# MaxRamgraber/Triangular-Transport-Toolbox

Hardware: AMD Instinct MI355X
Metric: map-evals/sec (forward+inverse, N samples x D comps) (higher is better)
Workload: dtype f64; 1 GPU; C5: d=40 banded separable map, order 3, N=1e6 (Gaussian-mixture target); N_per_gpu=1000000, D=40, columns=40, inverse=table, layout=column-major resident in HBM, coefficients=reference-optimised (tests/golden), world_size=1

## Files before the change

### triangular_transport_toolbox_amd/build.py

```python
import hashlib
import os
import shlex
import shutil
import subprocess

PKG = os.path.dirname(os.path.abspath(__file__))
CSRC = os.path.join(PKG, 'csrc')
LIB = os.environ.get('TTM_BUILD_LIB') or os.path.join(PKG, 'libttm.so')
SOURCES = ['ttm_kernels.hip', 'ttm_band.hip', 'ttm_int.hip', 'ttm_optim.cpp', 'ttm_comm.cpp']
HEADERS = ['ttm_eval.h', 'ttm_math.h', 'ttm_vec.h', 'ttm_erf_table.h', 'ttm_uform.h', 'ttm_cheb_table.h', 'ttm_lbfgsb.h', 'ttm_bfgs.h', 'ttm_rng.h', 'ttm_band.h', 'ttm_band_etab.h', 'ttm_dev.h', 'ttm_dense.h', 'ttm_dense_table.h', 'ttm_int.h', 'ttm_xprog.h', 'ttm_handover.h', 'ttm_options.h',
           os.path.join('..', '..', 'include', 'ttm.h')]
FLAGS = ['-O3', '-std=c++17', '--offload-arch=gfx950', '-ffp-contract=off', '-fPIC', '-shared',
         '-DNDEBUG'] + shlex.split(os.environ.get('TTM_BUILD_FLAGS', ''))
LINK = ['-ldl', '-pthread']


def hipcc_path():
    for cand in (shutil.which('hipcc'), '/opt/rocm/bin/hipcc'):
        if cand and os.path.exists(cand):
            return cand
    raise RuntimeError('hipcc not found: the MI355X engine needs the ROCm toolchain to build libttm.so')


def _sources():
    return [os.path.join(CSRC, s) for s in SOURCES if os.path.exists(os.path.join(CSRC, s))]
# ... 96 lines not shown
```

### triangular_transport_toolbox_amd/csrc/ttm_band.h

```cpp
#pragma once

#include <stdint.h>

#include "../../include/ttm.h"

namespace ttm_band {

int build_records(const ttm_program* p, double* U, void* stream);

int record_stride(int cls, int lag);

bool usable(const ttm_program* p, int k0, int k1);

int forward(const ttm_program* p, const double* U, int k0, int k1, const double* Xsoa, int64_t ldx, int64_t N, double* Zsoa,
            int64_t ldz, double* logdet, const double* sigma, double* sumsq, int cus, size_t lds_per_cu, int block, void* stream, const char** kernel_name);

int inverse(const ttm_program* p, const double* U, int k0, int k1, const double* Zsoa, int64_t ldz, double* Xsoa, int64_t ldx,
            int64_t N, const double* tab_x, int T, const double* y_affine, const double* tmin, const double* tmax, const int32_t* bkt,
            int nb, const double* img, int img_doubles, int cus, size_t lds_per_cu, int window, int block, void* stream, const char** kernel_name);

int newton(const ttm_program* p, const double* U, int k0, int k1, const double* Zsoa, int64_t ldz, double* Xsoa, int64_t ldx, int64_t N,
           int32_t* iters, int cus, size_t lds_per_cu, int block, void* stream, const char** kernel_name);

int bisect(const ttm_program* p, const double* U, int k0, int k1, const double* Zsoa, int64_t ldz, double* Xsoa, int64_t ldx, int64_t N,
           int32_t* iters, int cus, size_t lds_per_cu, int block, void* stream, const char** kernel_name);

bool bisect_plans(const ttm_program* p, const double* U, int k0, int k1, const double* Zsoa, int64_t ldz, double* Xsoa, int64_t ldx, int64_t N,
                  int32_t* iters, int cus, size_t lds_per_cu, int block);

int roundtrip(const ttm_program* p, const double* U, int k0, int k1, const double* Xsoa, int64_t ldx, int64_t N, double* Zsoa, int64_t ldz,
              double* Xr, int64_t ldr, double* logdet, const double* sigma, double* sumsq, const double* tab_x, int T, const double* y_affine,
              const double* tmin, const double* tmax, const int32_t* bkt, int nb, int cus, size_t lds_per_cu, bool force, void* stream,
              const char** kernel_name);

// ... 6 lines not shown
```

### triangular_transport_toolbox_amd/csrc/ttm_band.hip

```cpp
#include <hip/hip_runtime.h>
#include <math.h>
#include <stdint.h>
#include <stdlib.h>
#include <type_traits>

#include "ttm_band.h"
#include "ttm_band_etab.h"
#include "ttm_band_image.h"

namespace ttm_band {

typedef const __attribute__((address_space(4))) double* cdbl_p;
typedef const __attribute__((address_space(4))) int* cint_p;
struct __attribute__((aligned(16))) D2 { double x, y; };

__device__ const double g_band_etab[2 * TTM_BAND_ET_N] = { TTM_BAND_ETAB_VALUES };
__device__ double g_band_taylor[6] = {1.0 / 5040.0, 1.0 / 720.0, 1.0 / 120.0, 1.0 / 24.0, 1.0 / 6.0, 0.5};

__host__ __device__ constexpr int cls_db(int cls) { return cls == 1 ? 3 : (cls == 2 ? 5 : (cls == 3 ? 7 : 10)); }
__host__ __device__ constexpr int cls_da(int cls) { return cls == 1 ? 1 : (cls == 2 ? 5 : (cls == 3 ? 7 : 10)); }
__host__ __device__ constexpr int cls_gs(int cls) { return cls == 1 ? 8 : (cls == 2 ? 16 : 24); }
__host__ __device__ constexpr int cls_gp(int cls) { return cls_db(cls) + 1 + cls_da(cls); }
__host__ __device__ constexpr int rec_stride(int cls, int lag) { return (TTM_P_HDR + lag * cls_gp(cls) + 7) / 8 * 8; }

#define BAND_ET_DOUBLES (2 * TTM_BAND_ET_N)
#define BAND_CT 1024
#define BAND_NS 4
#define BAND_PF 1

__device__ __forceinline__ void band_dma16(const void* g, unsigned int lds_wave_base) {
    asm volatile("s_mov_b32 m0, %1\n\ts_nop 0\n\tglobal_load_lds_dwordx4 %0, off" ::"v"(g), "s"(lds_wave_base) : "m0");
}
__device__ __forceinline__ unsigned int band_lds_addr(const void* p) {
    return (unsigned int)(uintptr_t)(const __attribute__((address_space(3))) void*)p;
}

template <bool WAIT = true>
__device__ __forceinline__ void band_stage(double* lds_dst, const double* src, int n) {
    const int units = n >> 1;
    const unsigned int base = band_lds_addr(lds_dst);
    for (int u0 = 0; u0 < units; u0 += BAND_CT) {
        const int u = u0 + (int)threadIdx.x;
        if (u < units) band_dma16(src + 2 * (size_t)u, __builtin_amdgcn_readfirstlane(base + (unsigned int)(u0 + ((int)threadIdx.x & ~63)) * 16u));
// ... 56 lines not shown
    if (k >= 0) {
        const double* h = hot(k);
        const int* uc = ucomp + k * TTM_UC_LEN;
        double* tab = U + uc[TTM_UC_TAB_OFF];
        for (int c = t; c < uc[TTM_UC_NI]; c += 64) tab[c * TTM_U_TSTRIDE + 12] = fma(2.0, h[3], -(double)(2 * c - 1));
    }
}

template <bool NT>
__device__ __forceinline__ void band_store2(char* p, double a, double b) {
    typedef double v2 __attribute__((ext_vector_type(2)));
    const v2 v = {a, b};
    if (NT) __builtin_nontemporal_store(v, (v2*)p);
    else *(v2*)p = v;
}
__device__ __forceinline__ D2 band_load2(const char* p) {
    typedef double v2 __attribute__((ext_vector_type(2)));
    const v2 v = *(const v2*)p;
    const D2 r = {v.x, v.y};
    return r;
}

__device__ __forceinline__ int band_med3(int v, int lo, int hi) {
    int r;
    asm("v_med3_i32 %0, %1, %2, %3" : "=v"(r) : "v"(v), "v"(lo), "s"(hi));
    return r;
}
__device__ __forceinline__ double band_absmin(double x, double hi) {
    double r;
    asm("v_min_f64 %0, |%1|, %2" : "=v"(r) : "v"(x), "s"(hi));
    return r;
}

__device__ __forceinline__ double band_expq(const double* etab, double x, cdbl_p kt) {
    const double xe = band_absmin(x, TTM_BAND_ET_XMAX);
    const unsigned int i = (unsigned int)(int)fma(xe, TTM_BAND_ET_INV_STEP, 0.5);
// ... 48 lines not shown
}

__device__ __forceinline__ double band_spline(const double* tab, int nI, double sp_a, double sp_b, double sp_ds, double x) {
    const int col = band_med3((int)fma(x, sp_b, sp_a), 0, nI - 1);
    const double* cp = (const double*)((const char*)tab + __umul24((unsigned int)col, TTM_U_TSTRIDE * 8));
    double c[12];
#pragma unroll
    for (int i = 0; i < 12; i += 2) { const D2 v = *(const D2*)(cp + i); c[i] = v.x; c[i + 1] = v.y; }
    const double s = fma(x, sp_ds, cp[12]);
    double m = c[11];
#pragma unroll
    for (int i = 10; i >= 0; --i) m = fma(m, s, c[i]);
    return m;
}

template <int CLS, int LAG, bool FULL, bool OWN>
__device__ __forceinline__ void band_forward_tile(cdbl_p P, cdbl_p kt, const double* etab, const double* tabs, int tab0, int kb, int ke,
                                                  const char* xcol, int64_t ldxb, char* zcol, int64_t ldzb, unsigned int tbase,
                                                  const unsigned int (&roff)[BAND_NS / 2], unsigned int c1_32,
                                                  double (&pend)[BAND_NS][LAG]) {
    constexpr int DB = cls_db(CLS), DA = cls_da(CLS), PS = rec_stride(CLS, LAG);
    constexpr int NS = BAND_NS, NP = NS / 2, HALF = 2 * BAND_CT;
    constexpr int PF = BAND_PF, RING = PF + 1;
    D2 xr[RING][NP];
#pragma unroll
    for (int i = 0; i < PF; ++i) {
        const char* xc0 = xcol + (int64_t)(kb + i < ke ? i : 0) * ldxb;
#pragma unroll
        for (int q = 0; q < NP; ++q) xr[i][q] = band_load2(xc0 + roff[q]);
    }
    cdbl_p rec = P + (int64_t)(kb + LAG) * PS;
    auto step = [&](int j, const D2 (&xc)[NP], D2 (&xn)[NP]) {
        {
            const char* xnext = j + PF < ke ? xcol + PF * ldxb : xcol;
#pragma unroll
            for (int q = 0; q < NP; ++q) xn[q] = band_load2(xnext + roff[q]);
        }
        __builtin_amdgcn_sched_barrier(0);
        const double start = rec[0], sp_a = rec[2], sp_b = rec[3], sp_ds = rec[4];
        const double own1 = OWN ? rec[7] : 0.0;
        cint_p ri = (cint_p)rec;
        const int nI = ri[10];
        const double* tab = tabs + (ri[11] - tab0);
#pragma unroll
        for (int q = 0; q < NP; ++q) {
            double zv[2];
#pragma unroll
            for (int h = 0; h < 2; ++h) {
                const int e = 2 * q + h;
                const double x = h ? xc[q].y : xc[q].x;
                const double m = (!OWN || nI > 0) ? band_spline(tab, nI, sp_a, sp_b, sp_ds, x) : 0.0;
                const double E = band_expq(etab, x, kt);
                zv[h] = OWN ? fma(own1, x, pend[e][0] + m) : pend[e][0] + m;
                band_push<DB, DA, LAG>(rec + TTM_P_HDR, start, x, E, pend[e]);
            }
            const unsigned int n = tbase + (unsigned int)(q * HALF);
            const D2 o = {zv[0], zv[1]};
            char* zp = zcol + (size_t)(n * 8u);
            if (FULL || n + 1 < c1_32) band_store2<false>(zp, o.x, o.y);
            else if (n < c1_32) *(double*)zp = o.x;
            __builtin_amdgcn_sched_barrier(0);
        }
        rec += PS; xcol += ldxb; zcol += ldzb;
    };
    int j = kb;
    for (; j + RING <= ke; j += RING) {
#pragma unroll
        for (int i = 0; i < RING; ++i) step(j + i, xr[i], xr[(i + PF) % RING]);
    }
#pragma unroll
    for (int i = 0; i < RING - 1; ++i)
        if (j + i < ke) step(j + i, xr[i], xr[(i + PF) % RING]);
}

__device__ __forceinline__ double band_log(double x) {
    int e;
// ... 397 lines not shown
                    lv[h] = fma((double)pexp[e], 6.93147180559945286e-01, band_log(prod[e]));
                    lv[h] = dmin[e] < 0.0 ? NAN : lv[h];
                    if (last) lv[h] += luni;
                }
                if (!first) {
                    if (n + 1 < c1_32) { const D2 o = *(const D2*)(logdet + n); lv[0] += o.x; lv[1] += o.y; }
                    else if (n < c1_32) lv[0] += logdet[n];
                }
                if (n + 1 < c1_32) band_store2<false>((char*)(logdet + n), lv[0], lv[1]);
                else if (n < c1_32) logdet[n] = lv[0];
            }
        }
    }
}

template <int CLS, int LAG, bool OWN>
__global__ __launch_bounds__(BAND_CT) void k_band_forward(const double* __restrict__ U_, int64_t p_off, int k0, int k1, int kcol0,
                                                          const double* __restrict__ X, int64_t ldx, int64_t N,
                                                          double* __restrict__ Z, int64_t ldz, int64_t rows_per_wg, int Bc) {
    constexpr int DB = cls_db(CLS), DA = cls_da(CLS), PS = rec_stride(CLS, LAG);
    constexpr int NS = BAND_NS, NP = NS / 2, CT = BAND_CT, ROWS = NS * CT, HALF = 2 * CT;
    extern __shared__ __align__(16) double g_lds[];
    double* etab = g_lds;
    double* tabs = g_lds + BAND_ET_DOUBLES;
    const int tid = threadIdx.x;
    const int64_t c0 = (int64_t)blockIdx.x * rows_per_wg;
    if (c0 >= N) return;
    const int64_t c1 = c0 + rows_per_wg < N ? c0 + rows_per_wg : N;
    const int ntile = (int)((c1 - c0 + ROWS - 1) / ROWS);
    band_stage<false>(etab, g_band_etab, 2 * TTM_BAND_ET_N);
    cdbl_p P = (cdbl_p)(U_ + p_off);
// ... 35 lines not shown
                for (int i = 0; i < LAG; ++i) {
                    const int cc = colb - LAG + i;
                    cdbl_p rec = P + (int64_t)(kb + i) * PS;
                    const char* col = (const char*)X + (int64_t)(cc < 0 ? 0 : cc) * ldxb;
#pragma unroll
                    for (int q = 0; q < NP; ++q) {
                        D2 xv = *(const D2*)(col + roff[q]);
                        if (cc < 0) { xv.x = 0.0; xv.y = 0.0; }
                        band_push<DB, DA, LAG>(rec + TTM_P_HDR, rec[0], xv.x, band_expq(etab, xv.x, kt), pend[2 * q]);
                        band_push<DB, DA, LAG>(rec + TTM_P_HDR, rec[0], xv.y, band_expq(etab, xv.y, kt), pend[2 * q + 1]);
                    }
                }
            }
            const char* xcol = (const char*)X + (int64_t)colb * ldxb;
            char* zcol = (char*)Z + (int64_t)(kb - k0) * ldzb;
            if (full) band_forward_tile<CLS, LAG, true, OWN>(P, kt, etab, tabs, tab0, kb, ke, xcol, ldxb, zcol, ldzb, tbase, roff, c1_32, pend);
            else band_forward_tile<CLS, LAG, false, OWN>(P, kt, etab, tabs, tab0, kb, ke, xcol, ldxb, zcol, ldzb, tbase, roff, c1_32, pend);
        }
    }
}

#define BAND_FEW_NS 2
#define BAND_FEW_TAB (4 * BAND_CT)
template <int CLS, int LAG, int LAGE, bool PLAIN, bool DENS>
__global__ __launch_bounds__(BAND_CT) void k_band_few(const double* __restrict__ U_, int64_t p_off, int k0, int k1, int kcol0,
                                                      const double* __restrict__ X, int64_t ldx, int64_t N,
                                                      double* __restrict__ Z, int64_t ldz, double* __restrict__ logdet,
                                                      const double* __restrict__ sigma, double* __restrict__ sumsq, int ntiles,
                                                      int tab0, int ntab) {
    constexpr int DB = cls_db(CLS), DA = cls_da(CLS), GP = cls_gp(CLS), PS = rec_stride(CLS, LAG);
    constexpr int NS = BAND_FEW_NS, NP = NS / 2, CT = BAND_CT, ROWS = NS * CT, HALF = 2 * CT, FD = TTM_P_FEW_D;
    extern __shared__ __align__(16) double g_lds[];
// ... 218 lines not shown
};

__device__ __forceinline__ void band_ring_fill(const double* img, int ncomp, double* tabs, int tab_slot, int n) {
    const int U = tab_slot >> 1;
    const int total = n * U;
    for (int u0 = 0; u0 < total; u0 += BAND_CT) {
        const int u = u0 + (int)threadIdx.x;
        if (u < total) {
            const int t = u / U, o = u - t * U;
            band_dma16(img + (size_t)(t % ncomp) * tab_slot + 2 * o,
                       __builtin_amdgcn_readfirstlane(band_lds_addr(tabs) + (unsigned int)(u0 + ((int)threadIdx.x & ~63)) * 16u));
        }
    }
}

template <int CLS, int LAG, bool RING = false, int G = 0>
__device__ __forceinline__ void band_inverse_tile(const BandInvCtx& cx, bool full, int kb, int ke, const char* zcol, char* xcol, unsigned int tbase,
                                                  const unsigned int (&roff)[BAND_NS / 2], double (&pend)[BAND_NS][LAG],
                                                  const D2 (&zfirst)[BAND_NS / 2], bool have_first, BandRing* rg = nullptr) {
    constexpr int DB = cls_db(CLS), DA = cls_da(CLS), PS = rec_stride(CLS, LAG);
    constexpr int NS = BAND_NS, NP = NS / 2, HALF = 2 * BAND_CT;
    cdbl_p rec = cx.P + (int64_t)(kb + LAG) * PS;
    cdbl_p kt = cx.kt;
    const double* slot = RING ? cx.tabs + (size_t)rg->pos * cx.tab_slot : cx.tabs;
    const double ystep = cx.ystep;
    const int nb1 = cx.nb - 1;
    D2 za[NP], zb[NP];
    if (have_first) {
#pragma unroll
        for (int q = 0; q < NP; ++q) za[q] = zfirst[q];
    } else {
#pragma unroll
        for (int q = 0; q < NP; ++q) za[q] = band_load2(zcol + roff[q]);
    }
    auto interp = [&](double y_lo, double x_lo, double x_hi, double e_lo, double tgt, double& rr, double& ee) {
        const double dx = fmax(x_hi - x_lo, 1e-300);
        double rc = __builtin_amdgcn_rcp(dx);
        rc = fma(fma(-dx, rc, 1.0), rc, rc);
        const double delta = (ystep * rc) * (tgt - x_lo);
        rr = delta + y_lo;
        const double w = (delta * -0.25) * (y_lo + rr);
        double p = fma(kt[0], w, kt[1]);
        p = fma(p, w, kt[2]);
        p = fma(p, w, kt[3]);
        p = fma(p, w, kt[4]);
        p = fma(p, w, kt[5]);
        p = fma(p, w, 1.0);
        p = fma(p, w, 1.0);
        ee = e_lo * p;
    };
    auto step = [&](int j, const D2 (&zc)[NP], D2 (&zn)[NP]) {
        {
            const char* znext = j + 1 < ke ? zcol + cx.ldzb : zcol;
#pragma unroll
            for (int q = 0; q < NP; ++q) zn[q] = band_load2(znext + roff[q]);
        }
        double start = rec[1];
        double gc[LAG * (DB + 1 + DA)];
#pragma unroll
        for (int i = 0; i < LAG * (DB + 1 + DA); ++i) gc[i] = rec[TTM_P_HDR + i];
        asm volatile("" : "+s"(start));
#pragma unroll
        for (int i = 0; i < LAG * (DB + 1 + DA); ++i) asm volatile("" : "+s"(gc[i]));
        __builtin_amdgcn_sched_barrier(0);
        double wl, wh, scale, bias;
        { const D2 a = *(const D2*)slot; wl = a.x; wh = a.y; const D2 b = *(const D2*)(slot + 2); scale = b.x; bias = b.y; }
        const lds_p xsl = band_lds(slot + BAND_RT_HDR) - 8 * cx.w0;
        const lds_p bkl = band_lds(slot + BAND_RT_HDR + cx.Weven);
        const bool deg = __builtin_amdgcn_readfirstlane(((const int*)slot)[10]) != 0;
        const int per = __builtin_amdgcn_readfirstlane(((const int*)slot)[8]);
// ... 55 lines not shown
                    int a = 0, b = cx.T;
                    while (a < b) {
                        const int mid = (a + b) >> 1;
                        if (xg[mid] < t) a = mid + 1; else b = mid;
                    }
                    const int i = min(max(a, 1), cx.T - 1);
                    interp(fma((double)i, ystep, cx.y0m), xg[i - 1], xg[i], band_expq_series((double)(i - 1) * ystep + cx.y0), t, r[e], E[e]);
                }
            }
        }
#pragma unroll
        for (int e = 0; e < NS; ++e) band_push<DB, DA, LAG>(gc, start, r[e], E[e], pend[e]);
        if (full) {
#pragma unroll
            for (int q = 0; q < NP; ++q) {
                band_store2<false>(xcol + (size_t)((tbase + (unsigned int)(q * HALF)) * 8u), r[2 * q], r[2 * q + 1]);
            }
        } else {
#pragma unroll
            for (int q = 0; q < NP; ++q) {
                const unsigned int n = tbase + (unsigned int)(q * HALF);
                const D2 o = {r[2 * q], r[2 * q + 1]};
                char* xp = xcol + (size_t)(n * 8u);
                if (n + 1 < cx.c1_32) *(D2*)xp = o;
                else if (n < cx.c1_32) *(double*)xp = o.x;
            }
        }
        rec += PS; slot += cx.tab_slot; zcol += cx.ldzb; xcol += cx.ldxb;
        if (RING) {
            if (++rg->pos == rg->R) { rg->pos = 0; slot = cx.tabs; }
            if (G > 0 && ++rg->gcnt == G) {
                rg->gcnt = 0;
                static_assert(G == 0 || G == 4, "the counted wait below is 3 G - 2");
                asm volatile("s_waitcnt vmcnt(10)" ::: "memory");
                __syncthreads();
            }
        }
    };
    int j = kb;
// ... 150 lines not shown
                    for (int q = 0; q < NP; ++q) {
                        D2 xv = {0.0, 0.0};
                        if (cc >= 0) xv = *(const D2*)(col + roff[q]);
                        band_push<DB, DA, LAG>(rec + TTM_P_HDR, rec[1], xv.x, cc >= 0 ? band_expq_series(xv.x) : 1.0, pend[2 * q]);
                        band_push<DB, DA, LAG>(rec + TTM_P_HDR, rec[1], xv.y, cc >= 0 ? band_expq_series(xv.y) : 1.0, pend[2 * q + 1]);
                    }
                }
            }
            const char* zcol = (const char*)Z + (int64_t)(kb - k0) * ldzb;
            char* xcol = (char*)X + (int64_t)colb * ldxb;
            band_inverse_tile<CLS, LAG>(cx, full, kb, ke, zcol, xcol, tbase, roff, pend, zfirst, tile == 0);
        }
    }
}

template <int CLS, int LAG, int G>
__global__ __launch_bounds__(BAND_CT) void k_band_inverse_ring(const double* __restrict__ U_, int64_t p_off, int k0, int k1, int kcol0,
                                                               const double* __restrict__ Z, int64_t ldz, double* X, int64_t ldx, int64_t N,
                                                               const double* __restrict__ tab_x, int T, double y0, double ystep, double ylast,
                                                               const double* __restrict__ tmin, const double* __restrict__ tmax,
                                                               const double* __restrict__ img, int nb, int tab_slot, int R,
                                                               int64_t rows_per_wg, int w0, int W) {
    constexpr int DB = cls_db(CLS), DA = cls_da(CLS), PS = rec_stride(CLS, LAG);
    constexpr int NS = BAND_NS, NP = NS / 2, CT = BAND_CT, ROWS = NS * CT, HALF = 2 * CT;
    extern __shared__ __align__(16) double g_lds[];
    const int tid = threadIdx.x;
    const int64_t c0 = (int64_t)blockIdx.x * rows_per_wg;
    if (c0 >= N) return;
    const int64_t c1 = c0 + rows_per_wg < N ? c0 + rows_per_wg : N;
    const int ntile = (int)((c1 - c0 + ROWS - 1) / ROWS);
    const int ncomp = k1 - k0;
// ... 12 lines not shown
    cx.y0 = y0; cx.ystep = ystep; cx.y0m = y0m; cx.ldzb = ldzb; cx.ldxb = ldxb; cx.c1_32 = (unsigned int)c1;
    BandRing rg;
    {
        const int U = tab_slot >> 1, nw = (U + 63) >> 6;
        const int piece = (tid >> 6) % nw;
        const int start = 64 * piece < U - 64 ? 64 * piece : U - 64;
        rg.src = (const char*)img + (size_t)(start + (tid & 63)) * 16;
        rg.dst = __builtin_amdgcn_readfirstlane((unsigned int)start * 16u);
        rg.tabs_lds = band_lds_addr(tabs);
        rg.stride = (unsigned int)tab_slot * 8u;
        rg.R = R; rg.ncomp = ncomp; rg.pos = 0; rg.gcnt = 0;
        rg.tpos = G > 0 ? R - G : 0;
        rg.tcomp = G > 0 ? (R - G) % ncomp : 0;
    }
    D2 zfirst[NP];
#pragma unroll
    for (int q = 0; q < NP; ++q) {
        unsigned int n = (unsigned int)c0 + 2u * (unsigned int)tid + (unsigned int)(q * HALF);
        n = n < last_pair ? n : last_pair;
        zfirst[q] = band_load2((const char*)Z + (size_t)(n * 8u));
    }
    band_ring_fill(img, ncomp, tabs, tab_slot, R);
    for (int i = tid; i < W; i += CT) {
        etab[2 * i] = band_expq_series(w0 + i == T - 1 ? ylast : (double)(w0 + i) * ystep + y0);
        etab[2 * i + 1] = fma((double)(w0 + i + 1), ystep, y0m);
    }
    asm volatile("s_waitcnt vmcnt(0)" ::: "memory");
    __syncthreads();
    for (int tile = 0; tile < ntile; ++tile) {
        const unsigned int tbase = (unsigned int)c0 + (unsigned int)tile * (unsigned int)ROWS + 2u * (unsigned int)tid;
        const bool full = c0 + (int64_t)(tile + 1) * ROWS <= c1;
        unsigned int roff[NP];
#pragma unroll
        for (int q = 0; q < NP; ++q) {
            unsigned int n = tbase + (unsigned int)(q * HALF);
            n = n < last_pair ? n : last_pair;
// ... 4 lines not shown
        for (int e = 0; e < NS; ++e)
#pragma unroll
            for (int l = 0; l < LAG; ++l) pend[e][l] = 0.0;
        for (int i = 0; i < LAG; ++i) {
            const int cc = kcol0 - LAG + i;
            cdbl_p rec = P + (int64_t)(k0 + i) * PS;
            const char* col = (const char*)X + (int64_t)(cc < 0 ? 0 : cc) * ldxb;
#pragma unroll
            for (int q = 0; q < NP; ++q) {
                D2 xv = {0.0, 0.0};
                if (cc >= 0) xv = *(const D2*)(col + roff[q]);
                band_push<DB, DA, LAG>(rec + TTM_P_HDR, rec[1], xv.x, cc >= 0 ? band_expq_series(xv.x) : 1.0, pend[2 * q]);
                band_push<DB, DA, LAG>(rec + TTM_P_HDR, rec[1], xv.y, cc >= 0 ? band_expq_series(xv.y) : 1.0, pend[2 * q + 1]);
            }
        }
        band_inverse_tile<CLS, LAG, true, G>(cx, full, k0, k1, (const char*)Z, (char*)X + (int64_t)kcol0 * ldxb, tbase, roff, pend, zfirst, tile == 0, &rg);
    }
}

template <int CLS, int LAG, int LAGE, bool PLAIN>
__global__ __launch_bounds__(BAND_CT) void k_band_few_inverse(const double* __restrict__ U_, int64_t p_off, int k0, int k1, int kcol0,
                                                              const double* __restrict__ Z, int64_t ldz, double* X, int64_t ldx, int64_t N,
                                                              const double* __restrict__ tab_x, int T, double y0, double ystep, double ylast,
                                                              const double* __restrict__ tmin, const double* __restrict__ tmax,
                                                              const int* __restrict__ bkt, int nb, int tab_slot, int ntiles) {
    constexpr int DB = cls_db(CLS), DA = cls_da(CLS), GP = cls_gp(CLS), PS = rec_stride(CLS, LAG);
    constexpr int NS = BAND_FEW_NS, NP = NS / 2, CT = BAND_CT, ROWS = NS * CT, HALF = 2 * CT, FD = TTM_P_FEW_D, HDR = BAND_RT_HDR;
    extern __shared__ __align__(16) double g_lds[];
    const int tid = threadIdx.x;
    const int nc = k1 - k0;
    const int Weven = (T + 4 + 1) & ~1;
// ... 1386 lines not shown
static size_t block_lds_span(const ttm_program* p, int k0, int k1, int Bc, bool splines_only) {
    size_t lds = 0;
    for (int kb = k0; kb < k1; kb += Bc) {
        int a = kb, b = (kb + Bc < k1 ? kb + Bc : k1) - 1;
        if (splines_only) {
            while (a <= b && uc(p, a, TTM_UC_NI) <= 0) ++a;
            while (b >= a && uc(p, b, TTM_UC_NI) <= 0) --b;
        }
        const size_t s = a > b ? 0 : (size_t)(uc(p, b, TTM_UC_TAB_OFF) + TTM_U_TSTRIDE * uc(p, b, TTM_UC_NI) - uc(p, a, TTM_UC_TAB_OFF)) * 8;
        lds = s > lds ? s : lds;
    }
    return lds;
}

int forward(const ttm_program* p, const double* U, int k0, int k1, const double* Xsoa, int64_t ldx, int64_t N, double* Zsoa, int64_t ldz,
            double* logdet, const double* sigma, double* sumsq, int cus, size_t lds_per_cu, int block, void* stream, const char** kernel_name) {
    if (!usable(p, k0, k1) || (!Zsoa && !logdet && !sumsq) || N >= ((int64_t)1 << 28)) return 1;
    if (!col_ok(Xsoa, ldx, even_rows(N)) || (Zsoa && !col_ok(Zsoa, ldz, 0)) || !vec_ok(U) || !vec_ok(logdet) || !vec_ok(sumsq)) return 1;
    const bool dens = logdet || sumsq;
    const size_t stat = dens ? (size_t)BAND_UNI * 8 : 0;
    if (dens && k1 - k0 > BAND_UNI) return 1;
    const size_t fixed = (size_t)BAND_ET_DOUBLES * 8 + stat;
    if (lds_per_cu <= fixed) return 1;
    const int Bc = plan_blocks(p, k0, k1, lds_per_cu - fixed, block);
    if (Bc <= 0) return 1;
    const size_t lds = block_lds_sum(p, k0, k1, Bc) + fixed - stat;
    const int cls = p->u_h_cls, lag = p->u_p_lag, kcol0 = uc(p, k0, TTM_UC_KC);
    if (logdet && !Zsoa && !sumsq && k1 - k0 <= BAND_UNI) {
        const size_t lbudget = lds_per_cu - (size_t)BAND_UNI * 8;
        const int LBc = plan_blocks(p, k0, k1, lbudget, block);
        const size_t llds = LBc > 0 ? block_lds_span(p, k0, k1, LBc, true) + 16 : 0;
// ... 23 lines not shown
                          ldx, N, Zsoa, ldz, logdet, sigma, sumsq, fs.ntiles, fs.tab0, fs.ntab);
        }
    }
    if (lag != 2 || cls > 3) return 1;
    const bool own = sweep_has_own(p, k0, k1);
    const ChunkGrid cg = chunk_grid(N, cus);
    if (dens) {
        auto dk = with_bool(Zsoa != nullptr, [&](auto WZ) {
            return with_bool(own, [&](auto OW) {
                return with_cls<3>(cls, [&](auto C) { return k_band_density<decltype(C)::value, 2, decltype(WZ)::value, decltype(OW)::value>; });
            });
        });
        return launch(dk, cg.grid, lds, stream, "k_band_density", kernel_name, U, p->u_p_off, k0, k1, kcol0, Xsoa, ldx, N, Zsoa, ldz, logdet, sigma,
                      sumsq, cg.rows, Bc);
    }
    auto kern = with_bool(own, [&](auto OW) { return with_cls<3>(cls, [&](auto C) { return k_band_forward<decltype(C)::value, 2, decltype(OW)::value>; }); });
    return launch(kern, cg.grid, lds, stream, "k_band_forward", kernel_name, U, p->u_p_off, k0, k1, kcol0, Xsoa, ldx, N, Zsoa, ldz, cg.rows, Bc);
}

int roundtrip(const ttm_program* p, const double* U, int k0, int k1, const double* Xsoa, int64_t ldx, int64_t N, double* Zsoa, int64_t ldz,
              double* Xr, int64_t ldr, double* logdet, const double* sigma, double* sumsq, const double* tab_x, int T, const double* y_affine,
              const double* tmin, const double* tmax, const int32_t* bkt, int nb, int cus, size_t lds_per_cu, bool force, void* stream,
              const char** kernel_name) {
    const int nc = k1 - k0;
    if (!usable(p, k0, k1) || nc > TTM_P_FEW_D || !Xr || T < 64 || T + 4 > BAND_CT || nb + 1 != 1024 || N >= ((int64_t)1 << 28)) return 1;
    if (!vec_ok(bkt) || (sigma && !logdet) || !y_affine_ok(y_affine)) return 1;
    const int64_t need = even_rows(N);
    if (!col_ok(Xsoa, ldx, need) || (Zsoa && !col_ok(Zsoa, ldz, need)) || !col_ok(Xr, ldr, need) || !vec_ok(U) || !vec_ok(logdet) || !vec_ok(sumsq))
        return 1;
    const FewSweep fs = few_sweep(p, k0, k1, N, cus);
    const BandImageSlot slot = band_image_slot(T, nb);
// ... 83 lines not shown
static BlockPlan block_plan(int T, int W, int nb, int ncomp, size_t lds_per_cu, int block) {
    const BandImageSlot slot = band_image_slot(W, nb);
    BlockPlan b = {W, (T - W) / 2, slot.tab_slot, 0, 0, 0};
    if (slot.lds(1) > lds_per_cu) return b;
    b.Bc = (int)((lds_per_cu - slot.lds(0)) / ((size_t)slot.tab_slot * 8));
    if (b.Bc > ncomp) b.Bc = ncomp;
    if (b.Bc > BAND_RT_KMAX) b.Bc = BAND_RT_KMAX;
    if (block > 0 && block < b.Bc) b.Bc = block;
    b.nblk = (ncomp + b.Bc - 1) / b.Bc;
    b.lds = slot.lds(b.Bc);
    return b;
}

int inverse(const ttm_program* p, const double* U, int k0, int k1, const double* Zsoa, int64_t ldz, double* Xsoa, int64_t ldx, int64_t N,
            const double* tab_x, int T, const double* y_affine, const double* tmin, const double* tmax, const int32_t* bkt, int nb, const double* img,
            int img_doubles, int cus, size_t lds_per_cu, int window, int block, void* stream, const char** kernel_name) {
    if (!usable(p, k0, k1) || T < 64 || T > 4096 || nb + 1 != 1024 || N >= ((int64_t)1 << 28)) return 1;
    if (!vec_ok(bkt) || !y_affine_ok(y_affine)) return 1;
    if (!col_ok(Zsoa, ldz, even_rows(N)) || !col_ok(Xsoa, ldx, even_rows(N))) return 1;
    const int ncomp = k1 - k0, cls = p->u_h_cls, lag = p->u_p_lag, kcol0 = uc(p, k0, TTM_UC_KC);
    if (ncomp <= TTM_P_FEW_D && T + 4 <= BAND_CT && window <= 0) {
        const BandImageSlot slot = band_image_slot(T, nb);
        const FewSweep fs = few_sweep(p, k0, k1, N, cus);
        if (slot.lds(ncomp) <= lds_per_cu && fs.lage <= lag) {
            auto fk = with_reach(lag, fs.lage, [&](auto L, auto E) {
                return with_bool(fs.plain, [&](auto PL) {
                    return with_cls<4>(cls, [&](auto C) {
                        return k_band_few_inverse<decltype(C)::value, decltype(L)::value, decltype(E)::value, decltype(PL)::value>;
                    });
                });
            });
            return launch(fk, fs.grid, slot.lds(ncomp), stream, "k_band_few_inverse", kernel_name, U, p->u_p_off, k0, k1, kcol0, Zsoa, ldz, Xsoa, ldx,
                          N, tab_x, T, y_affine[0], y_affine[1], y_affine[2], tmin, tmax, bkt, nb, slot.tab_slot, fs.ntiles);
        }
    }
    if (lag != 2 || cls > 3) return 1;
    const ChunkGrid cg = chunk_grid(N, cus);
    BandRingPlan pl;
    if (img && vec_ok(img) && band_ring_plan(T, nb, ncomp, lds_per_cu, window, block, BAND_WFRAC, &pl) &&
        pl.tab_slot == img_doubles) {
        auto rk = with_bool(pl.G == 4, [&](auto G4) {
            return with_cls<3>(cls, [&](auto C) { return k_band_inverse_ring<decltype(C)::value, 2, decltype(G4)::value ? 4 : 0>; });
        });
        return launch(rk, cg.grid, pl.lds, stream, "k_band_inverse_ring", kernel_name, U, p->u_p_off, k0, k1, kcol0, Zsoa, ldz, Xsoa, ldx, N, tab_x, T,
                      y_affine[0], y_affine[1], y_affine[2], tmin, tmax, img, nb, pl.tab_slot, pl.R, cg.rows, pl.w0, pl.W);
    }
    BlockPlan b = block_plan(T, T, nb, ncomp, lds_per_cu, block);
    if (window != 0 && (window > 0 || (b.Bc > 0 && b.nblk > 1))) {
        int W = window > 0 ? (window < 16 ? 16 : window) : (int)(BAND_WFRAC * T);
        if (W >= T) W = T - 1;
        const BlockPlan w = block_plan(T, W, nb, ncomp, lds_per_cu, block);
        if (w.Bc > 0 && (window > 0 || w.nblk < b.nblk)) b = w;
    }
    if (b.Bc <= 0) return 1;
    auto kern = with_cls<3>(cls, [&](auto C) { return k_band_inverse<decltype(C)::value, 2, BAND_RT_KMAX>; });
    return launch(kern, cg.grid, b.lds, stream, "k_band_inverse", kernel_name, U, p->u_p_off, k0, k1, kcol0, Zsoa, ldz, Xsoa, ldx, N, tab_x, T,
                  y_affine[0], y_affine[1], y_affine[2], tmin, tmax, bkt, nb, b.tab_slot, b.Bc, cg.rows, b.w0, b.W);
// ... 9 lines not shown
```

### triangular_transport_toolbox_amd/csrc/ttm_kernels.hip

```cpp

#include <hip/hip_runtime.h>
#include <mutex>

#include <stdio.h>
#include <stdlib.h>
#include <string.h>

#include <type_traits>

#include "ttm_eval.h"
#include "ttm_dev.h"
#include "ttm_dense.h"
#include "ttm_rng.h"
#include "ttm_uform.h"
#include "ttm_band.h"
#include "ttm_band_image.h"
#include "ttm_int.h"
#include "ttm_options.h"

using namespace ttm;


static thread_local char g_err[512] = "";

// ... 2915 lines not shown
        const int chunk = (k1 - k0 + nchunk - 1) / nchunk;
        if (ibd && ttm_int::forward(p, dev_prog(p), k0, k1, coef, fold, Xsoa, ldx, N, Zsoa, ldz, logdet, sigma, sumsq, tiles, chunk, ibd,
                                    lds_bytes(nsl, ibd, 0, 1), tuning().int_xprog != 0, stream, &name) == TTM_OK)
            return check_launch(name);
    }
    if (sep && u_on(p) && all_fast(p, k0, k1) && N < ((int64_t)1 << 29)) {
        int tab_cap = 0;
        for (int k = k0; k < k1; ++k) {
            const int c = TTM_U_TSTRIDE * p->h_ucomp[k * TTM_UC_LEN + TTM_UC_NI];
            tab_cap = c > tab_cap ? c : tab_cap;
        }
        const int ways = plan_ways_of(p);
        if (band_forward_gate(p, k0, k1, N)) {
            const char* name = nullptr;
            if (ttm_band::forward(p, fold + fold_base_size(p), k0, k1, Xsoa, ldx, N, Zsoa, ldz, logdet, sigma, sumsq, band_cus(),
                                  device_info().lds_per_cu, tuning().rt_block, stream, &name) == 0)
                return check_launch(name);
        }
        {
            int nimax = 0, nchmax = 0;
            for (int k = k0; k < k1; ++k) {
                const int ni = p->h_ucomp[k * TTM_UC_LEN + TTM_UC_NI];
                nimax = ni > nimax ? ni : nimax;
            }
            nchmax = (nimax * TTM_U_TSTRIDE * 8 + 1023) >> 10;
            const int tab_slot = TTM_U_TSTRIDE * nimax;
            int xlead = 3, tlead = 2;
            const Tuning& tn = tuning();
            int hNS = 4;
            if (tn.hl_ns > 0) hNS = tn.hl_ns == 4 ? 4 : 2;
            const bool hot = hot_sweepable(p) && !tn.u_no_hot;
// ... 245 lines not shown
                      int64_t ldz, double* Xsoa, int64_t ldx, int64_t N, const double* tab_x, const double* tab_y, int64_t ldy,
                      int32_t T, const double* h_y_affine, const double* tmin, const double* tmax, const int32_t* bkt, int32_t nb,
                      int32_t truncate, const double* img, int64_t img_doubles, void* stream) {
    int rc = validate(p, k0, k1);
    if (rc) return rc;
    if (!coef || !fold || !Zsoa || !Xsoa || !tab_x || !tab_y || !tmin || !tmax || !bkt || N < 1 || ldx < N || ldz < N || T < 2 ||
        T < 8 || T > 65536 || nb < 4 || nb > 65536 || (ldy != 0 && ldy < T) || (h_y_affine && ldy != 0))
        return set_err(TTM_E_ARG, "ttm_inverse_table: bad arguments%s");
    if (p->monotonicity != TTM_MONO_SEPARABLE) return set_err(TTM_E_UNSUPPORTED, "table inverse needs separable monotonicity%s");
    const Tuning& tn = tuning();
    const bool affine = h_y_affine && ldy == 0;
    if (affine && truncate && band_inverse_gate(p, k0, k1, N, T, nb)) {
        const char* name = nullptr;
        if (ttm_band::inverse(p, fold + fold_base_size(p), k0, k1, Zsoa, ldz, Xsoa, ldx, N, tab_x, (int)T, h_y_affine, tmin, tmax, bkt, (int)nb,
                              tn.band_ring != 0 ? img : nullptr, (int)img_doubles, band_cus(), device_info().lds_per_cu, tn.rt_window, tn.rt_block,
                              stream, &name) == 0)
            return check_launch(name);
    }
    if (affine && rt_inverse_gate(p, k0, k1, N, T, nb) && hot_sweepable(p) && (k1 - k0 >= 4 || tn.u_loader == 1)) {
        const DeviceInfo& di = device_info();
        const int ways = plan_ways_of(p);
        const int ncomp = k1 - k0;
        int NS = tn.rt_ns == 4 ? 4 : 2;
        int W = T, w0 = 0;
        int Weven = (W + 4 + 1) & ~1;
        int tab_slot = TTM_RT_HDR + Weven + (((nb + 1 + 3) / 4 + 1) & ~1);
        const double ymax = fabs(h_y_affine[0]) > fabs(h_y_affine[2]) ? fabs(h_y_affine[0]) : fabs(h_y_affine[2]);
        const bool etab = truncate && h_y_affine[1] > 0.0 && h_y_affine[1] * ymax * 0.5 <= 0.1;
        const bool aligned = ((uintptr_t)Zsoa % 16 == 0) && (ldz % 2 == 0) && ldz >= ((N + 1) & ~(int64_t)1) &&
                             ((uintptr_t)Xsoa % 16 == 0) && (ldx % 2 == 0) && ldx >= ((N + 1) & ~(int64_t)1);
        bool band = p->u_h_ng == 2 && tn.rt_band != 0;
// ... 508 lines not shown
```

### triangular_transport_toolbox_amd/csrc/ttm_options.h

```cpp
#pragma once

#include <string.h>

#define TTM_OPTIONS(X)                                                                                                   \
    X(no_plan, 0)         \
    X(no_uform, 0)        \
    X(u_no_hot, 0)        \
    X(u_loader, -1)       \
    X(forward_ns, -1)     \
    X(inverse_ns, -1)     \
    X(u_ns, -1)           \
    X(hl_ns, -1)          \
    X(rt_off, 0)          \
    X(rt_ns, -1)          \
    X(rt_block, -1)       \
    X(rt_band, -1)        \
    X(rt_window, -1)      \
    X(gram_mfma, -1)      \
    X(band_fwd, -1)       \
    X(band_inv, -1)       \
    X(band_cus, -1)       \
    X(band_ring, -1)      \
    X(band_newton, -1)    \
    X(band_bisect, -1)    \
    X(int_dense, -1)      \
    X(int_xprog, -1)      \
    X(fold_fused, -1)     \
    X(table_fused, -1)    \
    X(setup_fused, -1)    \
    X(select_coop, -1)    \
    X(colstats_one, -1)   \
    X(sep_sentinel, -1)   \
    X(sep_server, -1)     \
    X(roundtrip_fused, -1)

struct Tuning {
#define X(name, dflt) int name = dflt;
    TTM_OPTIONS(X)
#undef X
// ... 9 lines not shown
```

Baseline: 157.2 billion map-evals/s.

## Keep half of Z resident in LLC across band forward and inverse

Adds a cache-residency policy for the banded forward and ring-inverse kernels. When the Z columns exceed the 256 MB last-level cache but the rows of pair slot 0 of each tile fit, the forward path uses nontemporal loads for X and nontemporal stores for the slot-1 Z rows. The slot-0 Z rows are stored normally, so they can stay cached and be re-read by the inverse, which also streams its X output nontemporally. The aim is to cut HBM traffic between the two stages, at the cost of more template instantiations and a policy that assumes a fixed LLC size.

```diff
diff --git a/triangular_transport_toolbox_amd/build.py b/triangular_transport_toolbox_amd/build.py
--- a/triangular_transport_toolbox_amd/build.py
+++ b/triangular_transport_toolbox_amd/build.py
@@ -8,7 +8,7 @@
 CSRC = os.path.join(PKG, 'csrc')
 LIB = os.environ.get('TTM_BUILD_LIB') or os.path.join(PKG, 'libttm.so')
 SOURCES = ['ttm_kernels.hip', 'ttm_band.hip', 'ttm_int.hip', 'ttm_optim.cpp', 'ttm_comm.cpp']
-HEADERS = ['ttm_eval.h', 'ttm_math.h', 'ttm_vec.h', 'ttm_erf_table.h', 'ttm_uform.h', 'ttm_cheb_table.h', 'ttm_lbfgsb.h', 'ttm_bfgs.h', 'ttm_rng.h', 'ttm_band.h', 'ttm_band_etab.h', 'ttm_dev.h', 'ttm_dense.h', 'ttm_dense_table.h', 'ttm_int.h', 'ttm_xprog.h', 'ttm_handover.h', 'ttm_options.h',
+HEADERS = ['ttm_eval.h', 'ttm_math.h', 'ttm_vec.h', 'ttm_erf_table.h', 'ttm_uform.h', 'ttm_cheb_table.h', 'ttm_lbfgsb.h', 'ttm_bfgs.h', 'ttm_rng.h', 'ttm_band.h', 'ttm_band_etab.h', 'ttm_band_policy.h', 'ttm_dev.h', 'ttm_dense.h', 'ttm_dense_table.h', 'ttm_int.h', 'ttm_xprog.h', 'ttm_handover.h', 'ttm_options.h',
            os.path.join('..', '..', 'include', 'ttm.h')]
 FLAGS = ['-O3', '-std=c++17', '--offload-arch=gfx950', '-ffp-contract=off', '-fPIC', '-shared',
          '-DNDEBUG'] + shlex.split(os.environ.get('TTM_BUILD_FLAGS', ''))
diff --git a/triangular_transport_toolbox_amd/csrc/ttm_band.h b/triangular_transport_toolbox_amd/csrc/ttm_band.h
--- a/triangular_transport_toolbox_amd/csrc/ttm_band.h
+++ b/triangular_transport_toolbox_amd/csrc/ttm_band.h
@@ -13,11 +13,13 @@
 bool usable(const ttm_program* p, int k0, int k1);
 
 int forward(const ttm_program* p, const double* U, int k0, int k1, const double* Xsoa, int64_t ldx, int64_t N, double* Zsoa,
-            int64_t ldz, double* logdet, const double* sigma, double* sumsq, int cus, size_t lds_per_cu, int block, void* stream, const char** kernel_name);
+            int64_t ldz, double* logdet, const double* sigma, double* sumsq, int cus, size_t lds_per_cu, int block, int resident, void* stream,
+            const char** kernel_name);
 
 int inverse(const ttm_program* p, const double* U, int k0, int k1, const double* Zsoa, int64_t ldz, double* Xsoa, int64_t ldx,
             int64_t N, const double* tab_x, int T, const double* y_affine, const double* tmin, const double* tmax, const int32_t* bkt,
-            int nb, const double* img, int img_doubles, int cus, size_t lds_per_cu, int window, int block, void* stream, const char** kernel_name);
+            int nb, const double* img, int img_doubles, int cus, size_t lds_per_cu, int window, int block, int resident, void* stream,
+            const char** kernel_name);
 
 int newton(const ttm_program* p, const double* U, int k0, int k1, const double* Zsoa, int64_t ldz, double* Xsoa, int64_t ldx, int64_t N,
            int32_t* iters, int cus, size_t lds_per_cu, int block, void* stream, const char** kernel_name);
diff --git a/triangular_transport_toolbox_amd/csrc/ttm_band.hip b/triangular_transport_toolbox_amd/csrc/ttm_band.hip
--- a/triangular_transport_toolbox_amd/csrc/ttm_band.hip
+++ b/triangular_transport_toolbox_amd/csrc/ttm_band.hip
@@ -3,10 +3,12 @@
 #include <stdint.h>
 #include <stdlib.h>
 #include <type_traits>
+#include <utility>
 
 #include "ttm_band.h"
 #include "ttm_band_etab.h"
 #include "ttm_band_image.h"
+#include "ttm_band_policy.h"
 
 namespace ttm_band {
 
@@ -27,6 +29,8 @@
 #define BAND_CT 1024
 #define BAND_NS 4
 #define BAND_PF 1
+static_assert(BAND_POLICY_TILE_ROWS == BAND_NS * BAND_CT && BAND_POLICY_HALF_ROWS == 2 * BAND_CT && BAND_NS == 4,
+              "ttm_band_policy.h counts the rows of pair slot 0 of these tiles");
 
 __device__ __forceinline__ void band_dma16(const void* g, unsigned int lds_wave_base) {
     asm volatile("s_mov_b32 m0, %1\n\ts_nop 0\n\tglobal_load_lds_dwordx4 %0, off" ::"v"(g), "s"(lds_wave_base) : "m0");
@@ -113,12 +117,20 @@
     if (NT) __builtin_nontemporal_store(v, (v2*)p);
     else *(v2*)p = v;
 }
+template <bool NT = false>
 __device__ __forceinline__ D2 band_load2(const char* p) {
     typedef double v2 __attribute__((ext_vector_type(2)));
-    const v2 v = *(const v2*)p;
+    v2 v;
+    if (NT) v = __builtin_nontemporal_load((const v2*)p);
+    else v = *(const v2*)p;
     const D2 r = {v.x, v.y};
     return r;
 }
+template <int POL, int Q> constexpr bool band_z_nt = POL != 0 && Q != 0;
+template <class F, int... Q>
+__device__ __forceinline__ void band_slots_seq(F& f, std::integer_sequence<int, Q...>) { (f(std::integral_constant<int, Q>{}), ...); }
+template <int N, class F>
+__device__ __forceinline__ void band_slots(F&& f) { band_slots_seq(f, std::make_integer_sequence<int, N>{}); }
 
 __device__ __forceinline__ int band_med3(int v, int lo, int hi) {
     int r;
@@ -197,7 +209,30 @@
     return m;
 }
 
-template <int CLS, int LAG, bool FULL, bool OWN>
+template <int CLS, int LAG, bool FULL, bool OWN, bool NT>
+__device__ __forceinline__ void band_forward_rows(int q, const D2 (&xc)[BAND_NS / 2], double (&pend)[BAND_NS][LAG], cdbl_p rec, double start, double sp_a,
+                                                  double sp_b, double sp_ds, double own1, int nI, const double* tab, const double* etab, cdbl_p kt,
+                                                  unsigned int tbase, char* zcol, unsigned int c1_32) {
+    constexpr int DB = cls_db(CLS), DA = cls_da(CLS), HALF = 2 * BAND_CT;
+    double zv[2];
+#pragma unroll
+    for (int h = 0; h < 2; ++h) {
+        const int e = 2 * q + h;
+        const double x = h ? xc[q].y : xc[q].x;
+        const double m = (!OWN || nI > 0) ? band_spline(tab, nI, sp_a, sp_b, sp_ds, x) : 0.0;
+        const double E = band_expq(etab, x, kt);
+        zv[h] = OWN ? fma(own1, x, pend[e][0] + m) : pend[e][0] + m;
+        band_push<DB, DA, LAG>(rec + TTM_P_HDR, start, x, E, pend[e]);
+    }
+    const unsigned int n = tbase + (unsigned int)(q * HALF);
+    const D2 o = {zv[0], zv[1]};
+    char* zp = zcol + (size_t)(n * 8u);
+    if (FULL || n + 1 < c1_32) band_store2<NT>(zp, o.x, o.y);
+    else if (n < c1_32) *(double*)zp = o.x;
+    __builtin_amdgcn_sched_barrier(0);
+}
+
+template <int CLS, int LAG, bool FULL, bool OWN, int POL = 0>
 __device__ __forceinline__ void band_forward_tile(cdbl_p P, cdbl_p kt, const double* etab, const double* tabs, int tab0, int kb, int ke,
                                                   const char* xcol, int64_t ldxb, char* zcol, int64_t ldzb, unsigned int tbase,
                                                   const unsigned int (&roff)[BAND_NS / 2], unsigned int c1_32,
@@ -210,14 +245,14 @@
     for (int i = 0; i < PF; ++i) {
         const char* xc0 = xcol + (int64_t)(kb + i < ke ? i : 0) * ldxb;
 #pragma unroll
-        for (int q = 0; q < NP; ++q) xr[i][q] = band_load2(xc0 + roff[q]);
+        for (int q = 0; q < NP; ++q) xr[i][q] = band_load2<POL != 0>(xc0 + roff[q]);
     }
     cdbl_p rec = P + (int64_t)(kb + LAG) * PS;
     auto step = [&](int j, const D2 (&xc)[NP], D2 (&xn)[NP]) {
         {
             const char* xnext = j + PF < ke ? xcol + PF * ldxb : xcol;
 #pragma unroll
-            for (int q = 0; q < NP; ++q) xn[q] = band_load2(xnext + roff[q]);
+            for (int q = 0; q < NP; ++q) xn[q] = band_load2<POL != 0>(xnext + roff[q]);
         }
         __builtin_amdgcn_sched_barrier(0);
         const double start = rec[0], sp_a = rec[2], sp_b = rec[3], sp_ds = rec[4];
@@ -225,24 +260,31 @@
         cint_p ri = (cint_p)rec;
         const int nI = ri[10];
         const double* tab = tabs + (ri[11] - tab0);
-#pragma unroll
-        for (int q = 0; q < NP; ++q) {
-            double zv[2];
-#pragma unroll
-            for (int h = 0; h < 2; ++h) {
-                const int e = 2 * q + h;
-                const double x = h ? xc[q].y : xc[q].x;
-                const double m = (!OWN || nI > 0) ? band_spline(tab, nI, sp_a, sp_b, sp_ds, x) : 0.0;
-                const double E = band_expq(etab, x, kt);
-                zv[h] = OWN ? fma(own1, x, pend[e][0] + m) : pend[e][0] + m;
-                band_push<DB, DA, LAG>(rec + TTM_P_HDR, start, x, E, pend[e]);
-            }
-            const unsigned int n = tbase + (unsigned int)(q * HALF);
-            const D2 o = {zv[0], zv[1]};
-            char* zp = zcol + (size_t)(n * 8u);
-            if (FULL || n + 1 < c1_32) band_store2<false>(zp, o.x, o.y);
-            else if (n < c1_32) *(double*)zp = o.x;
-            __builtin_amdgcn_sched_barrier(0);
+        if constexpr (POL == 0) {
+#pragma unroll
+            for (int q = 0; q < NP; ++q) {
+                double zv[2];
+#pragma unroll
+                for (int h = 0; h < 2; ++h) {
+                    const int e = 2 * q + h;
+                    const double x = h ? xc[q].y : xc[q].x;
+                    const double m = (!OWN || nI > 0) ? band_spline(tab, nI, sp_a, sp_b, sp_ds, x) : 0.0;
+                    const double E = band_expq(etab, x, kt);
+                    zv[h] = OWN ? fma(own1, x, pend[e][0] + m) : pend[e][0] + m;
+                    band_push<DB, DA, LAG>(rec + TTM_P_HDR, start, x, E, pend[e]);
+                }
+                const unsigned int n = tbase + (unsigned int)(q * HALF);
+                const D2 o = {zv[0], zv[1]};
+                char* zp = zcol + (size_t)(n * 8u);
+                if (FULL || n + 1 < c1_32) band_store2<false>(zp, o.x, o.y);
+                else if (n < c1_32) *(double*)zp = o.x;
+                __builtin_amdgcn_sched_barrier(0);
+            }
+        } else {
+            band_slots<NP>([&](auto Q) {
+                constexpr int q = decltype(Q)::value;
+                band_forward_rows<CLS, LAG, FULL, OWN, band_z_nt<POL, q>>(q, xc, pend, rec, start, sp_a, sp_b, sp_ds, own1, nI, tab, etab, kt, tbase, zcol, c1_32);
+            });
         }
         rec += PS; xcol += ldxb; zcol += ldzb;
     };
@@ -670,7 +712,7 @@
     }
 }
 
-template <int CLS, int LAG, bool OWN>
+template <int CLS, int LAG, bool OWN, int POL = 0>
 __global__ __launch_bounds__(BAND_CT) void k_band_forward(const double* __restrict__ U_, int64_t p_off, int k0, int k1, int kcol0,
                                                           const double* __restrict__ X, int64_t ldx, int64_t N,
                                                           double* __restrict__ Z, int64_t ldz, int64_t rows_per_wg, int Bc) {
@@ -736,8 +778,8 @@
             }
             const char* xcol = (const char*)X + (int64_t)colb * ldxb;
             char* zcol = (char*)Z + (int64_t)(kb - k0) * ldzb;
-            if (full) band_forward_tile<CLS, LAG, true, OWN>(P, kt, etab, tabs, tab0, kb, ke, xcol, ldxb, zcol, ldzb, tbase, roff, c1_32, pend);
-            else band_forward_tile<CLS, LAG, false, OWN>(P, kt, etab, tabs, tab0, kb, ke, xcol, ldxb, zcol, ldzb, tbase, roff, c1_32, pend);
+            if (full) band_forward_tile<CLS, LAG, true, OWN, POL>(P, kt, etab, tabs, tab0, kb, ke, xcol, ldxb, zcol, ldzb, tbase, roff, c1_32, pend);
+            else band_forward_tile<CLS, LAG, false, OWN, POL>(P, kt, etab, tabs, tab0, kb, ke, xcol, ldxb, zcol, ldzb, tbase, roff, c1_32, pend);
         }
     }
 }
@@ -986,7 +1028,7 @@
     }
 }
 
-template <int CLS, int LAG, bool RING = false, int G = 0>
+template <int CLS, int LAG, bool RING = false, int G = 0, int POL = 0>
 __device__ __forceinline__ void band_inverse_tile(const BandInvCtx& cx, bool full, int kb, int ke, const char* zcol, char* xcol, unsigned int tbase,
                                                   const unsigned int (&roff)[BAND_NS / 2], double (&pend)[BAND_NS][LAG],
                                                   const D2 (&zfirst)[BAND_NS / 2], bool have_first, BandRing* rg = nullptr) {
@@ -1002,8 +1044,7 @@
 #pragma unroll
         for (int q = 0; q < NP; ++q) za[q] = zfirst[q];
     } else {
-#pragma unroll
-        for (int q = 0; q < NP; ++q) za[q] = band_load2(zcol + roff[q]);
+        band_slots<NP>([&](auto Q) { constexpr int q = decltype(Q)::value; za[q] = band_load2<band_z_nt<POL, q>>(zcol + roff[q]); });
     }
     auto interp = [&](double y_lo, double x_lo, double x_hi, double e_lo, double tgt, double& rr, double& ee) {
         const double dx = fmax(x_hi - x_lo, 1e-300);
@@ -1024,8 +1065,7 @@
     auto step = [&](int j, const D2 (&zc)[NP], D2 (&zn)[NP]) {
         {
             const char* znext = j + 1 < ke ? zcol + cx.ldzb : zcol;
-#pragma unroll
-            for (int q = 0; q < NP; ++q) zn[q] = band_load2(znext + roff[q]);
+            band_slots<NP>([&](auto Q) { constexpr int q = decltype(Q)::value; zn[q] = band_load2<band_z_nt<POL, q>>(znext + roff[q]); });
         }
         double start = rec[1];
         double gc[LAG * (DB + 1 + DA)];
@@ -1111,7 +1151,7 @@
         if (full) {
 #pragma unroll
             for (int q = 0; q < NP; ++q) {
-                band_store2<false>(xcol + (size_t)((tbase + (unsigned int)(q * HALF)) * 8u), r[2 * q], r[2 * q + 1]);
+                band_store2<POL != 0>(xcol + (size_t)((tbase + (unsigned int)(q * HALF)) * 8u), r[2 * q], r[2 * q + 1]);
             }
         } else {
 #pragma unroll
@@ -1119,7 +1159,7 @@
                 const unsigned int n = tbase + (unsigned int)(q * HALF);
                 const D2 o = {r[2 * q], r[2 * q + 1]};
                 char* xp = xcol + (size_t)(n * 8u);
-                if (n + 1 < cx.c1_32) *(D2*)xp = o;
+                if (n + 1 < cx.c1_32) { if (POL != 0) band_store2<true>(xp, o.x, o.y); else *(D2*)xp = o; }
                 else if (n < cx.c1_32) *(double*)xp = o.x;
             }
         }
@@ -1300,7 +1340,7 @@
     }
 }
 
-template <int CLS, int LAG, int G>
+template <int CLS, int LAG, int G, int POL = 0>
 __global__ __launch_bounds__(BAND_CT) void k_band_inverse_ring(const double* __restrict__ U_, int64_t p_off, int k0, int k1, int kcol0,
                                                                const double* __restrict__ Z, int64_t ldz, double* X, int64_t ldx, int64_t N,
                                                                const double* __restrict__ tab_x, int T, double y0, double ystep, double ylast,
@@ -1343,12 +1383,12 @@
         rg.tcomp = G > 0 ? (R - G) % ncomp : 0;
     }
     D2 zfirst[NP];
-#pragma unroll
-    for (int q = 0; q < NP; ++q) {
+    band_slots<NP>([&](auto Q) {
+        constexpr int q = decltype(Q)::value;
         unsigned int n = (unsigned int)c0 + 2u * (unsigned int)tid + (unsigned int)(q * HALF);
         n = n < last_pair ? n : last_pair;
-        zfirst[q] = band_load2((const char*)Z + (size_t)(n * 8u));
-    }
+        zfirst[q] = band_load2<band_z_nt<POL, q>>((const char*)Z + (size_t)(n * 8u));
+    });
     band_ring_fill(img, ncomp, tabs, tab_slot, R);
     for (int i = tid; i < W; i += CT) {
         etab[2 * i] = band_expq_series(w0 + i == T - 1 ? ylast : (double)(w0 + i) * ystep + y0);
@@ -1383,7 +1423,7 @@
                 band_push<DB, DA, LAG>(rec + TTM_P_HDR, rec[1], xv.y, cc >= 0 ? band_expq_series(xv.y) : 1.0, pend[2 * q + 1]);
             }
         }
-        band_inverse_tile<CLS, LAG, true, G>(cx, full, k0, k1, (const char*)Z, (char*)X + (int64_t)kcol0 * ldxb, tbase, roff, pend, zfirst, tile == 0, &rg);
+        band_inverse_tile<CLS, LAG, true, G, POL>(cx, full, k0, k1, (const char*)Z, (char*)X + (int64_t)kcol0 * ldxb, tbase, roff, pend, zfirst, tile == 0, &rg);
     }
 }
 
@@ -2800,7 +2840,8 @@
 }
 
 int forward(const ttm_program* p, const double* U, int k0, int k1, const double* Xsoa, int64_t ldx, int64_t N, double* Zsoa, int64_t ldz,
-            double* logdet, const double* sigma, double* sumsq, int cus, size_t lds_per_cu, int block, void* stream, const char** kernel_name) {
+            double* logdet, const double* sigma, double* sumsq, int cus, size_t lds_per_cu, int block, int resident, void* stream,
+            const char** kernel_name) {
     if (!usable(p, k0, k1) || (!Zsoa && !logdet && !sumsq) || N >= ((int64_t)1 << 28)) return 1;
     if (!col_ok(Xsoa, ldx, even_rows(N)) || (Zsoa && !col_ok(Zsoa, ldz, 0)) || !vec_ok(U) || !vec_ok(logdet) || !vec_ok(sumsq)) return 1;
     const bool dens = logdet || sumsq;
@@ -2854,7 +2895,12 @@
         return launch(dk, cg.grid, lds, stream, "k_band_density", kernel_name, U, p->u_p_off, k0, k1, kcol0, Xsoa, ldx, N, Zsoa, ldz, logdet, sigma,
                       sumsq, cg.rows, Bc);
     }
-    auto kern = with_bool(own, [&](auto OW) { return with_cls<3>(cls, [&](auto C) { return k_band_forward<decltype(C)::value, 2, decltype(OW)::value>; }); });
+    const bool pol = (band_resident_policy(N, cg.rows, k1 - k0, resident) & BAND_POLICY_FORWARD) != 0;
+    auto kern = with_bool(pol, [&](auto PO) {
+        return with_bool(own, [&](auto OW) {
+            return with_cls<3>(cls, [&](auto C) { return k_band_forward<decltype(C)::value, 2, decltype(OW)::value, decltype(PO)::value ? 1 : 0>; });
+        });
+    });
     return launch(kern, cg.grid, lds, stream, "k_band_forward", kernel_name, U, p->u_p_off, k0, k1, kcol0, Xsoa, ldx, N, Zsoa, ldz, cg.rows, Bc);
 }
 
@@ -2968,7 +3014,7 @@
 
 int inverse(const ttm_program* p, const double* U, int k0, int k1, const double* Zsoa, int64_t ldz, double* Xsoa, int64_t ldx, int64_t N,
             const double* tab_x, int T, const double* y_affine, const double* tmin, const double* tmax, const int32_t* bkt, int nb, const double* img,
-            int img_doubles, int cus, size_t lds_per_cu, int window, int block, void* stream, const char** kernel_name) {
+            int img_doubles, int cus, size_t lds_per_cu, int window, int block, int resident, void* stream, const char** kernel_name) {
     if (!usable(p, k0, k1) || T < 64 || T > 4096 || nb + 1 != 1024 || N >= ((int64_t)1 << 28)) return 1;
     if (!vec_ok(bkt) || !y_affine_ok(y_affine)) return 1;
     if (!col_ok(Zsoa, ldz, even_rows(N)) || !col_ok(Xsoa, ldx, even_rows(N))) return 1;
@@ -2993,8 +3039,13 @@
     BandRingPlan pl;
     if (img && vec_ok(img) && band_ring_plan(T, nb, ncomp, lds_per_cu, window, block, BAND_WFRAC, &pl) &&
         pl.tab_slot == img_doubles) {
-        auto rk = with_bool(pl.G == 4, [&](auto G4) {
-            return with_cls<3>(cls, [&](auto C) { return k_band_inverse_ring<decltype(C)::value, 2, decltype(G4)::value ? 4 : 0>; });
+        const bool pol = (band_resident_policy(N, cg.rows, ncomp, resident) & BAND_POLICY_INVERSE) != 0;
+        auto rk = with_bool(pol, [&](auto PO) {
+            return with_bool(pl.G == 4, [&](auto G4) {
+                return with_cls<3>(cls, [&](auto C) {
+                    return k_band_inverse_ring<decltype(C)::value, 2, decltype(G4)::value ? 4 : 0, decltype(PO)::value ? 1 : 0>;
+                });
+            });
         });
         return launch(rk, cg.grid, pl.lds, stream, "k_band_inverse_ring", kernel_name, U, p->u_p_off, k0, k1, kcol0, Zsoa, ldz, Xsoa, ldx, N, tab_x, T,
                       y_affine[0], y_affine[1], y_affine[2], tmin, tmax, img, nb, pl.tab_slot, pl.R, cg.rows, pl.w0, pl.W);
diff --git a/triangular_transport_toolbox_amd/csrc/ttm_band_policy.h b/triangular_transport_toolbox_amd/csrc/ttm_band_policy.h
--- /dev/null
+++ b/triangular_transport_toolbox_amd/csrc/ttm_band_policy.h
@@ -0,0 +1,29 @@
+#pragma once
+
+#include <stdint.h>
+
+constexpr int64_t TTM_LLC_BYTES = (int64_t)256 << 20;
+
+constexpr int BAND_POLICY_TILE_ROWS = 4096;
+constexpr int BAND_POLICY_HALF_ROWS = 2048;
+
+constexpr int BAND_POLICY_FORWARD = 1;
+constexpr int BAND_POLICY_INVERSE = 2;
+
+static inline int64_t band_policy_resident_rows(int64_t N, int64_t chunk_rows) {
+    if (N <= 0 || chunk_rows <= 0) return 0;
+    auto of_chunk = [](int64_t n) {
+        const int64_t tail = n % BAND_POLICY_TILE_ROWS;
+        return n / BAND_POLICY_TILE_ROWS * BAND_POLICY_HALF_ROWS + (tail < BAND_POLICY_HALF_ROWS ? tail : BAND_POLICY_HALF_ROWS);
+    };
+    const int64_t whole = N / chunk_rows;
+    return whole * of_chunk(chunk_rows) + of_chunk(N - whole * chunk_rows);
+}
+
+static inline int band_resident_policy(int64_t N, int64_t chunk_rows, int ncomp, int option) {
+    if (option >= 0) return option & (BAND_POLICY_FORWARD | BAND_POLICY_INVERSE);
+    const int64_t col = 8 * (int64_t)ncomp;
+    if (col * N <= TTM_LLC_BYTES) return 0;
+    if (band_policy_resident_rows(N, chunk_rows) * col > TTM_LLC_BYTES) return 0;
+    return BAND_POLICY_FORWARD | BAND_POLICY_INVERSE;
+}
diff --git a/triangular_transport_toolbox_amd/csrc/ttm_kernels.hip b/triangular_transport_toolbox_amd/csrc/ttm_kernels.hip
--- a/triangular_transport_toolbox_amd/csrc/ttm_kernels.hip
+++ b/triangular_transport_toolbox_amd/csrc/ttm_kernels.hip
@@ -2953,7 +2953,7 @@
         if (band_forward_gate(p, k0, k1, N)) {
             const char* name = nullptr;
             if (ttm_band::forward(p, fold + fold_base_size(p), k0, k1, Xsoa, ldx, N, Zsoa, ldz, logdet, sigma, sumsq, band_cus(),
-                                  device_info().lds_per_cu, tuning().rt_block, stream, &name) == 0)
+                                  device_info().lds_per_cu, tuning().rt_block, tuning().band_resident, stream, &name) == 0)
                 return check_launch(name);
         }
         {
@@ -3229,7 +3229,7 @@
         const char* name = nullptr;
         if (ttm_band::inverse(p, fold + fold_base_size(p), k0, k1, Zsoa, ldz, Xsoa, ldx, N, tab_x, (int)T, h_y_affine, tmin, tmax, bkt, (int)nb,
                               tn.band_ring != 0 ? img : nullptr, (int)img_doubles, band_cus(), device_info().lds_per_cu, tn.rt_window, tn.rt_block,
-                              stream, &name) == 0)
+                              tn.band_resident, stream, &name) == 0)
             return check_launch(name);
     }
     if (affine && rt_inverse_gate(p, k0, k1, N, T, nb) && hot_sweepable(p) && (k1 - k0 >= 4 || tn.u_loader == 1)) {
diff --git a/triangular_transport_toolbox_amd/csrc/ttm_options.h b/triangular_transport_toolbox_amd/csrc/ttm_options.h
--- a/triangular_transport_toolbox_amd/csrc/ttm_options.h
+++ b/triangular_transport_toolbox_amd/csrc/ttm_options.h
@@ -23,6 +23,7 @@
     X(band_ring, -1)      \
     X(band_newton, -1)    \
     X(band_bisect, -1)    \
+    X(band_resident, -1)  \
     X(int_dense, -1)      \
     X(int_xprog, -1)      \
     X(fold_fused, -1)     \
```

Result: faster. 169.5 billion map-evals/s, median of 6 (+7.8%).
